# haliphinx/TCE-RVOS

Measured on AMD Instinct MI355X. Metric: clips/s (T=5, 360×640, Swin-T) at 1/2/4/8 MI355X; mask IoU vs ref, higher is better.
Workload: dtype f32 (3xf16-split MFMA, f32 accumulate); 1 GPU; swin_t_p4w7 T=5 360x640 + 32-token text, B=1 clip per forward, flags --with_box_refine --binary --f_token 8 --qtrans (BASELINE config 2); clips_in_flight_per_gpu=1, clips_per_forward=1, same_clip_in_group=False, ranks_per_gpu=1, parallelism=clip-sharded x1

## Files before the change

tce-rvos_amd/csrc/fewrow.hip:

```cpp
#include "common.h"
#include "../../include/tce_rvos.h"

namespace {

constexpr int FR_COLS = 8;
constexpr int FR_KC = 256;
constexpr int FR_PITCH = FR_KC + 4;

struct FrSegDev {
  const float* W;
  const float* bias;
  float* out;
  int N, ldw, ldo, use_a2, act, slab0;
};

struct FrArgs {
  const float* x;
  const float* a2;
  const float* res;
  long long ldx, lda2, ldres;
  int a2_rows, R, K, nseg;
  FrSegDev seg[3];
  const float *g_in, *be_in;
  float* xn_out;
  long long ldxn;
  float eps_in;
};

template <int RPT>
__global__ void __launch_bounds__(256) fewrow_linear_kernel(const FrArgs p) {
  __shared__ __attribute__((aligned(16))) float sX[32 * RPT * FR_PITCH];
  __shared__ __attribute__((aligned(16))) float sW[FR_COLS * FR_PITCH];
  const int tid = threadIdx.x;
  int s = 0;
  if (p.nseg > 1 && (int)blockIdx.x >= p.seg[1].slab0) s = 1;
  if (p.nseg > 2 && (int)blockIdx.x >= p.seg[2].slab0) s = 2;
  const FrSegDev sg = s == 0 ? p.seg[0] : (s == 1 ? p.seg[1] : p.seg[2]);
  const int n0 = ((int)blockIdx.x - sg.slab0) * FR_COLS;
  const int r0 = blockIdx.y * (32 * RPT);
  const int nr = min(32 * RPT, p.R - r0);
  const int c = tid & 7, g = tid >> 3;
  float acc[RPT];
#pragma unroll
  for (int i = 0; i < RPT; ++i) acc[i] = 0.f;
  for (int k0 = 0; k0 < p.K; k0 += FR_KC) {
    const int kc = min(FR_KC, p.K - k0);
    const int q4 = kc >> 2;
    if (k0) __syncthreads();
    if ((tid & 63) < q4) {
      const int q = tid & 63;
      for (int r = tid >> 6; r < 32 * RPT; r += 4) {
        f32x4 v = {0.f, 0.f, 0.f, 0.f};
        if (r < nr) {
          v = *reinterpret_cast<const f32x4*>(p.x + (long long)(r0 + r) * p.ldx + k0 + 4 * q);
          if (p.g_in) {
            const float mean = wave_sum((v[0] + v[1]) + (v[2] + v[3])) / (float)p.K;
            const f32x4 d = {v[0] - mean, v[1] - mean, v[2] - mean, v[3] - mean};
            const float rstd = rsqrtf(wave_sum(fmaf(d[0], d[0], fmaf(d[1], d[1], fmaf(d[2], d[2], d[3] * d[3])))) / (float)p.K + p.eps_in);
            const f32x4 g = *reinterpret_cast<const f32x4*>(p.g_in + 4 * q), b = *reinterpret_cast<const f32x4*>(p.be_in + 4 * q);
            v = f32x4{d[0] * rstd * g[0] + b[0], d[1] * rstd * g[1] + b[1], d[2] * rstd * g[2] + b[2], d[3] * rstd * g[3] + b[3]};
            if (p.xn_out && blockIdx.x == 0) *reinterpret_cast<f32x4*>(p.xn_out + (long long)(r0 + r) * p.ldxn + 4 * q) = v;
          }
          if (sg.use_a2) {
            const int ra = p.a2_rows > 0 ? (r0 + r) % p.a2_rows : r0 + r;
            v += *reinterpret_cast<const f32x4*>(p.a2 + (long long)ra * p.lda2 + k0 + 4 * q);
          }
        }
        *reinterpret_cast<f32x4*>(&sX[r * FR_PITCH + 4 * q]) = v;
      }
      for (int r = tid >> 6; r < FR_COLS; r += 4) {
        f32x4 v = {0.f, 0.f, 0.f, 0.f};
        if (n0 + r < sg.N) v = *reinterpret_cast<const f32x4*>(sg.W + (long long)(n0 + r) * sg.ldw + k0 + 4 * q);
        *reinterpret_cast<f32x4*>(&sW[r * FR_PITCH + 4 * q]) = v;
      }
    }
    __syncthreads();
    const float* wrow = &sW[c * FR_PITCH];
    const float* xrow = &sX[g * FR_PITCH];
    if (q4 == 64) {
#pragma unroll 8
      for (int q = 0; q < 64; ++q) {
        const f32x4 wv = *reinterpret_cast<const f32x4*>(wrow + 4 * q);
#pragma unroll
        for (int i = 0; i < RPT; ++i) {
          const f32x4 xv = *reinterpret_cast<const f32x4*>(xrow + i * 32 * FR_PITCH + 4 * q);
          acc[i] = fmaf(xv[0], wv[0], acc[i]);
          acc[i] = fmaf(xv[1], wv[1], acc[i]);
          acc[i] = fmaf(xv[2], wv[2], acc[i]);
          acc[i] = fmaf(xv[3], wv[3], acc[i]);
        }
      }
    } else {
      for (int q = 0; q < q4; ++q) {
        const f32x4 wv = *reinterpret_cast<const f32x4*>(wrow + 4 * q);
#pragma unroll
        for (int i = 0; i < RPT; ++i) {
          const f32x4 xv = *reinterpret_cast<const f32x4*>(xrow + i * 32 * FR_PITCH + 4 * q);
          acc[i] = fmaf(xv[0], wv[0], acc[i]);
          acc[i] = fmaf(xv[1], wv[1], acc[i]);
          acc[i] = fmaf(xv[2], wv[2], acc[i]);
          acc[i] = fmaf(xv[3], wv[3], acc[i]);
        }
      }
    }
  }
  const int n = n0 + c;
  if (n < sg.N) {
    const float bv = sg.bias ? sg.bias[n] : 0.f;
#pragma unroll
    for (int i = 0; i < RPT; ++i) {
      const int r = g + 32 * i;
      if (r < nr) {
        float v = acc[i] + bv;
        if (sg.act == 1) v = fmaxf(v, 0.f);
        if (sg.act == 2) v = 1.0f / (1.0f + __expf(-v));
        if (sg.act == 3) v = tce_gelu(v);
        if (s == 0 && p.res) v += p.res[(long long)(r0 + r) * p.ldres + n];
        sg.out[(long long)(r0 + r) * sg.ldo + n] = v;
      }
    }
  }
}

}

extern "C" int tce_fewrow_linear_f32(const tceFewRowArgs* a, tceStream stream) {
  TCE_CHECK_ARG(a && a->x && a->nseg >= 1 && a->nseg <= 3, "tce_fewrow_linear_f32: bad arguments");
  TCE_CHECK_ARG(a->R > 0 && a->K > 0 && a->K % 4 == 0 && a->ldx % 4 == 0 && a->ldx >= a->K && tce_aligned16(a->x),
                "tce_fewrow_linear_f32: K and ldx must be multiples of 4, ldx >= K, x 16-byte aligned");
  auto span = [&](const float* p, long long ld, long long cols, long long rows, const float*& b, const float*& e) {
    b = p;
    e = p + (rows - 1) * ld + cols;
  };
  auto disjoint = [](const float* b0, const float* e0, const float* b1, const float* e1) { return e0 <= b1 || e1 <= b0; };
  FrArgs p;
  p.g_in = a->g_in; p.be_in = a->be_in; p.xn_out = a->g_in ? a->xn_out : nullptr; p.ldxn = a->ldxn; p.eps_in = a->eps_in;
  if (a->g_in) {
    TCE_CHECK_ARG(a->be_in && a->K == FR_KC && tce_aligned16(a->g_in) && tce_aligned16(a->be_in),
                  "tce_fewrow_linear_f32: the LayerNorm prologue needs K = %d and 16-byte aligned gamma / beta", FR_KC);
    TCE_CHECK_ARG(!a->xn_out || (a->ldxn >= a->K && a->ldxn % 4 == 0 && tce_aligned16(a->xn_out)), "tce_fewrow_linear_f32: xn_out pitch / alignment");
  }
  p.x = a->x; p.a2 = a->a2; p.res = a->res;
  p.ldx = a->ldx; p.lda2 = a->lda2; p.ldres = a->ldres;
  p.a2_rows = a->a2_rows; p.R = a->R; p.K = a->K; p.nseg = a->nseg;
  int slabs = 0;
  for (int s = 0; s < 3; ++s) {
    FrSegDev& d = p.seg[s];
    d = FrSegDev{nullptr, nullptr, nullptr, 0, 0, 0, 0, 0, 1 << 30};
    if (s >= a->nseg) continue;
    const tceFewRowSeg& g = a->seg[s];
    TCE_CHECK_ARG(g.W && g.out && g.N > 0 && g.ldw % 4 == 0 && g.ldw >= a->K && g.ldo >= g.N && tce_aligned16(g.W),
                  "tce_fewrow_linear_f32: segment %d: bad weight / output geometry", s);
    TCE_CHECK_ARG(!g.use_a2 || (a->a2 && a->lda2 % 4 == 0 && tce_aligned16(a->a2)), "tce_fewrow_linear_f32: addend missing / misaligned");
    TCE_CHECK_ARG(g.act >= 0 && g.act <= 3, "tce_fewrow_linear_f32: act must be 0 (none), 1 (ReLU), 2 (sigmoid) or 3 (GELU)");
    {
      const float *xb, *xe, *ob, *oe;
      span(a->x, a->ldx, a->K, a->R, xb, xe);
      span(g.out, g.ldo, g.N, a->R, ob, oe);
      TCE_CHECK_ARG(disjoint(xb, xe, ob, oe), "tce_fewrow_linear_f32: segment %d: out overlaps x", s);
      if (a->a2) {
        const float *ab, *ae;
        span(a->a2, a->lda2, a->K, a->a2_rows > 0 ? a->a2_rows : a->R, ab, ae);
        TCE_CHECK_ARG(disjoint(ab, ae, ob, oe), "tce_fewrow_linear_f32: segment %d: out overlaps a2", s);
      }
      for (int t = 0; t < s; ++t) {
        const float *pb, *pe;
        span(a->seg[t].out, a->seg[t].ldo, a->seg[t].N, a->R, pb, pe);
        TCE_CHECK_ARG(disjoint(pb, pe, ob, oe), "tce_fewrow_linear_f32: outputs of segments %d and %d overlap", t, s);
      }
      if (a->g_in && a->xn_out) {
        const float *nb, *ne;
        span(a->xn_out, a->ldxn, a->K, a->R, nb, ne);
        TCE_CHECK_ARG(disjoint(nb, ne, xb, xe) && disjoint(nb, ne, ob, oe), "tce_fewrow_linear_f32: xn_out overlaps x or segment %d's out", s);
        if (a->a2) {
          const float *ab, *ae;
          span(a->a2, a->lda2, a->K, a->a2_rows > 0 ? a->a2_rows : a->R, ab, ae);
          TCE_CHECK_ARG(disjoint(nb, ne, ab, ae), "tce_fewrow_linear_f32: xn_out overlaps a2");
        }
      }
      if (a->res) {
        const float *rb, *re;
        span(a->res, a->ldres, a->seg[0].N, a->R, rb, re);
        const bool in_place = s == 0 && a->res == g.out && a->ldres == g.ldo;
        TCE_CHECK_ARG(in_place || disjoint(rb, re, ob, oe),
                      "tce_fewrow_linear_f32: segment %d: res overlaps out (only segment 0 may alias it, exactly)", s);
      }
    }
    d.W = g.W; d.bias = g.bias; d.out = g.out; d.N = g.N; d.ldw = g.ldw; d.ldo = g.ldo; d.use_a2 = g.use_a2; d.act = g.act;
    d.slab0 = slabs;
    slabs += tce_cdiv(g.N, FR_COLS);
  }
  TCE_CHECK_ARG(!a->res || a->ldres >= a->seg[0].N, "tce_fewrow_linear_f32: residual pitch");
#ifdef FEWROW_RPT2
  if (a->R > 32 && a->R <= 64) {
    hipLaunchKernelGGL(fewrow_linear_kernel<2>, dim3(slabs, 1), dim3(256), 0, (hipStream_t)stream, p);
    TCE_CHECK_LAUNCH("tce_fewrow_linear_f32");
    return TCE_OK;
  }
#endif
  hipLaunchKernelGGL(fewrow_linear_kernel<1>, dim3(slabs, tce_cdiv(a->R, 32)), dim3(256), 0, (hipStream_t)stream, p);
  TCE_CHECK_LAUNCH("tce_fewrow_linear_f32");
  return TCE_OK;
}
```

tce-rvos_amd/csrc/ffn.hip:

```cpp
#include "common.h"
#include "gemm_epilogue.h"
#include "frag.h"
#include "tiles.h"
#include "../../include/tce_rvos.h"
#include "../../include/tce_rvos_debug.h"

namespace {

#ifndef FFN_ABL
#define FFN_ABL 0
#endif
static __device__ long long* g_ffn_stamps = nullptr;

__device__ __forceinline__ void partial_store(const f32x16& acc, float* __restrict__ base, const int t, const int lane) {
#pragma unroll
  for (int g = 0; g < 4; ++g) {
    const f32x4 o = {acc[4 * g], acc[4 * g + 1], acc[4 * g + 2], acc[4 * g + 3]};
    float* const ptr = base + ((t * 4 + g) * 64 + lane) * 4;
    asm volatile("global_store_dwordx4 %0, %1, off sc1" ::"v"(ptr), "v"(o) : "memory");
  }
}
struct PartTile {
  f32x4 v[4];
};
// ... 429 lines not shown
    o = __builtin_bit_cast(u32x4, plane ? f.lo : f.hi);
  }
  reinterpret_cast<u32x4*>(out)[u] = o;
}

inline bool ffn_shape_ok(int C, int Hd) { return (C == 96 || C == 128 || C == 192 || C == 256) && Hd > 0 && Hd % 32 == 0; }
inline int ffn_waves(int C) { return C <= 128 ? 8 : 4; }
inline int ffn_pieces(int C) {
  const int w = ffn_waves(C);
  return (1 + 2 * (C / 16) + 4 * (C / 32) + w - 1) / w * w;
}
inline long long ffn_units(int C, int Hd) { return (long long)(Hd / 32 + 2) * ffn_pieces(C) * 64; }

struct FfnSplitPlan {
  int p = 0, k[2] = {0, 0}, nblk = 0;
  long long ws_floats = 0;
};
inline FfnSplitPlan ffn_split_plan(int M, int C, int Hd, int batch) {
  FfnSplitPlan best;
  const int B = tce_cdiv(M, 32 * ffn_waves(C)), NC = Hd / 32, CUS = tce_cu_count();
  if (C != 256 || NC < 24 || batch < 1) return best;
  const int OVP = 3, OVF = 4;
  auto rounds = [&](long long wgs) { return (double)((wgs + CUS - 1) / CUS); };
  double best_cost = 0.75 * rounds((long long)B * batch) * (NC + 1 + OVP + OVF);
  for (int p = 1; p <= 2; ++p) {
    const int wd = p == 1 ? 0 : (p * NC - 2 * (1 + OVP)) / (p + 1), ws_ = p == 1 ? (NC + 1) / 2 : wd + 1 + OVP;
    int k[2] = {ws_, 0};
    bool ok = ws_ >= 1 && ws_ <= NC - 1;
    for (int i = 1; i < p && ok; ++i) {
      k[i] = wd - (NC - k[i - 1]);
      ok = k[i] >= 1 && k[i] <= NC - 1;
    }
    if (!ok) continue;
    const int busiest = ws_ > NC - k[p - 1] ? ws_ : NC - k[p - 1];
    const double cost = rounds((long long)tce_cdiv(B, p) * (p + 1) * batch) * (busiest + 1 + OVP + OVF);
    if (cost < best_cost) {
      best_cost = cost;
      best.p = p;
      for (int i = 0; i < 2; ++i) best.k[i] = k[i];
    }
  }
  if (best.p) {
    best.nblk = B;
    best.ws_floats = (long long)batch * B * 2 * (32 * ffn_waves(C)) * C;
  }
  return best;
}

static int g_ffn_half = 0;

struct FfnGridPlan {
  int grid_x, persist;
};
inline FfnGridPlan ffn_grid_plan(int cap, int batch, int blocks) {
  if (cap <= 0 || batch < 1 || (long long)blocks * batch <= cap) return {blocks, 0};
  const int gx = cap / batch > 1 ? cap / batch : 1;
  if (gx >= blocks) return {blocks, 0};
  return {gx, 1};
}
static thread_local int t_ffn_wg_cap = 0;

template <int C, int WAVES>
void ffn_launch(const FfnArgs& a, int act, hipStream_t s, int batch = 1) {
  if constexpr (C == 256) {
    if (a.sp_p > 0 && act == 1) {
      const dim3 grid(tce_cdiv(a.nblk, a.sp_p) * (a.sp_p + 1), batch), block(64 * WAVES);
      if (a.single) hipLaunchKernelGGL((ffn_fused_kernel<C, WAVES, 1, true, 0, true>), grid, block, 0, s, a);
      else hipLaunchKernelGGL((ffn_fused_kernel<C, WAVES, 1, false, 0, true>), grid, block, 0, s, a);
      return;
    }
  }
  if constexpr (C <= 128 && WAVES == 8) {
    const long long b8 = (long long)tce_cdiv(a.M, 256) * batch, b4 = (long long)tce_cdiv(a.M, 128) * batch, cus = tce_cu_count();
    const double c8 = (double)((b8 + cus - 1) / cus);
    const long long rem = b4 % (2 * cus);
    const double c4 = (double)(b4 / (2 * cus)) + (rem == 0 ? 0.0 : rem <= cus ? 0.5 : 1.0);
    if (act == 2 && g_ffn_half >= 0 && (g_ffn_half > 0 || c4 <= c8)) {
      const dim3 grid(tce_cdiv(a.M, 128), batch), block(256);
      if (a.single) hipLaunchKernelGGL((ffn_fused_kernel<C, 4, 2, true>), grid, block, 0, s, a);
      else hipLaunchKernelGGL((ffn_fused_kernel<C, 4, 2, false>), grid, block, 0, s, a);
      return;
    }
  }
  if constexpr (C == 256) {
    const FfnGridPlan gp = ffn_grid_plan(t_ffn_wg_cap, batch, tce_cdiv(a.M, 32 * WAVES));
    if (gp.persist && act == 1) {
      const dim3 grid(gp.grid_x, batch), block(64 * WAVES);
      if (a.single) hipLaunchKernelGGL((ffn_fused_kernel<C, WAVES, 1, true, 0, false, true>), grid, block, 0, s, a);
      else hipLaunchKernelGGL((ffn_fused_kernel<C, WAVES, 1, false, 0, false, true>), grid, block, 0, s, a);
      return;
    }
  }
  const dim3 grid(tce_cdiv(a.M, 32 * WAVES), batch), block(64 * WAVES);
  if (a.single) {
    if (act == 1) hipLaunchKernelGGL((ffn_fused_kernel<C, WAVES, 1, true>), grid, block, 0, s, a);
    else if (act == 2) hipLaunchKernelGGL((ffn_fused_kernel<C, WAVES, 2, true>), grid, block, 0, s, a);
  } else {
    if (act == 1) hipLaunchKernelGGL((ffn_fused_kernel<C, WAVES, 1, false>), grid, block, 0, s, a);
    else if (act == 2) hipLaunchKernelGGL((ffn_fused_kernel<C, WAVES, 2, false>), grid, block, 0, s, a);
  }
}

__global__ void __launch_bounds__(256) xattn_prepare_kernel(const float* __restrict__ k, const float* __restrict__ v,
                                                            const float* __restrict__ wqT, const float* __restrict__ wo,
                                                            float* __restrict__ W1, float* __restrict__ b1,
                                                            float* __restrict__ W2, const int L, const int G,
                                                            const int* __restrict__ lens) {
  constexpr int C = 256, HD = 32;
  const int Hd = 8 * G;
  const int Lb = lens ? min(lens[blockIdx.y], L) : L;
  k += (long long)blockIdx.y * L * C;
  v += (long long)blockIdx.y * L * C;
  W1 += (long long)blockIdx.y * Hd * C;
  b1 += (long long)blockIdx.y * Hd;
  W2 += (long long)blockIdx.y * C * Hd;
  const int idx = blockIdx.x * 256 + threadIdx.x;
  if (idx < Hd * C) {
    const int r = idx / C, i = idx - r * C, h = r / G, j = r - h * G;
    float a = 0.f;
    if (j < Lb) {
      const f32x4* kp = reinterpret_cast<const f32x4*>(k + j * C + h * HD);
      const f32x4* wp = reinterpret_cast<const f32x4*>(wqT + (long long)i * C + h * HD);
#pragma unroll
      for (int c4 = 0; c4 < 8; ++c4) {
        const f32x4 kv = kp[c4], wv = wp[c4];
        a = fmaf(kv[0], wv[0], a); a = fmaf(kv[1], wv[1], a); a = fmaf(kv[2], wv[2], a); a = fmaf(kv[3], wv[3], a);
      }
    }
    W1[idx] = a;
  } else if (idx < 2 * Hd * C) {
    const int e = idx - Hd * C, n = e / Hd, r = e - n * Hd, h = r / G, j = r - h * G;
    float a = 0.f;
    if (j < Lb) {
      const f32x4* vp = reinterpret_cast<const f32x4*>(v + j * C + h * HD);
      const f32x4* wp = reinterpret_cast<const f32x4*>(wo + (long long)n * C + h * HD);
#pragma unroll
      for (int c4 = 0; c4 < 8; ++c4) {
        const f32x4 vv = vp[c4], wv = wp[c4];
        a = fmaf(vv[0], wv[0], a); a = fmaf(vv[1], wv[1], a); a = fmaf(vv[2], wv[2], a); a = fmaf(vv[3], wv[3], a);
      }
    }
    W2[e] = a;
  } else if (idx < 2 * Hd * C + Hd) {
    const int r = idx - 2 * Hd * C, h = r / G, j = r - h * G;
    float a = -1.0e30f;
    if (j < Lb) {
      a = 0.f;
      for (int c = 0; c < HD; ++c) a = fmaf(k[j * C + h * HD + c], wqT[(long long)C * C + h * HD + c], a);
    }
    b1[r] = a;
  }
}

__global__ void __launch_bounds__(256) xattn_pack_fused_kernel(const float* __restrict__ k, const float* __restrict__ v,
                                                               const float* __restrict__ wqT, const float* __restrict__ wo,
                                                               unsigned char* __restrict__ out, const int L, const int G,
                                                               const int P, const int SL, const long long threads,
                                                               const long long units, const int single,
                                                               const int* __restrict__ lens) {
  constexpr int C = 256, HD = 32, KS = C / 16, NT = C / 32;
  const long long tix = (long long)blockIdx.x * 256 + threadIdx.x;
  if (tix >= threads) return;
  const int Hd = 8 * G, NC = Hd / 32;
  const int Lb = lens ? min(lens[blockIdx.y], L) : L;
  k += (long long)blockIdx.y * L * C;
  v += (long long)blockIdx.y * L * C;
  out += (long long)blockIdx.y * units * 16;
  const int lane = (int)(tix & 63);
  const long long sg = tix >> 6;
  const int sl = (int)(sg % SL), it = (int)(sg / SL);
  const int r = lane & 31, hf = lane >> 5;
  u32x4* const stage_out = reinterpret_cast<u32x4*>(out) + (long long)it * P * 64;
  auto dot32 = [](const float* a, const float* b) {
    const f32x4* ap = reinterpret_cast<const f32x4*>(a);
    const f32x4* bp = reinterpret_cast<const f32x4*>(b);
    float acc = 0.f;
#pragma unroll
    for (int c4 = 0; c4 < 8; ++c4) {
      const f32x4 x = ap[c4], y = bp[c4];
      acc = fmaf(x[0], y[0], acc); acc = fmaf(x[1], y[1], acc); acc = fmaf(x[2], y[2], acc); acc = fmaf(x[3], y[3], acc);
    }
    return acc;
  };
  if (sl == 0) {
    u32x4 o = {0u, 0u, 0u, 0u};
    if (lane < 8 && it < NC) {
      f32x4 val;
#pragma unroll
      for (int c = 0; c < 4; ++c) {
        const int idx = 4 * lane + c, h2 = idx >> 4, i = idx & 15;
        const int row = 32 * it + (i & 3) + 8 * (i >> 2) + 4 * h2, h = row / G, j = row - h * G;
        float a = -1.0e30f;
        if (j < Lb) {
          a = 0.f;
          for (int c2 = 0; c2 < HD; ++c2) a = fmaf(k[j * C + h * HD + c2], wqT[(long long)C * C + h * HD + c2], a);
        }
        val[c] = a;
      }
      o = __builtin_bit_cast(u32x4, val);
    }
    stage_out[lane] = o;
    return;
  }
  const int p_hi = 2 * sl - 1, p_lo = 2 * sl;
  if (p_hi >= P) return;
  u32x4 oh = {0u, 0u, 0u, 0u}, ol = oh;
  if (p_hi < 1 + 2 * KS + 4 * NT) {
    float val[8];
    if (p_hi <= 2 * KS) {
      const int s = (p_hi - 1) >> 1;
      const int row = 32 * it + r, h = row / G, j = row - h * G;
#pragma unroll
      for (int e = 0; e < 8; ++e)
        val[e] = (it < NC && j < Lb) ? dot32(k + j * C + h * HD, wqT + (long long)(16 * s + 8 * hf + e) * C + h * HD) : 0.f;
    } else {
      const int idx = (p_hi - 1 - 2 * KS) >> 1, t = idx >> 1, s2 = idx & 1, chunk = it - 1;
#pragma unroll
      for (int e = 0; e < 8; ++e) {
        const int col = 32 * chunk + 16 * s2 + 8 * (e >> 2) + 4 * hf + (e & 3);
        const int h = col / G, j = col - h * G;
        val[e] = (chunk >= 0 && chunk < NC && j < Lb) ? dot32(wo + (long long)(32 * t + r) * C + h * HD, v + j * C + h * HD) : 0.f;
      }
    }
    const HL f = split8(val, single);
    oh = __builtin_bit_cast(u32x4, f.hi);
    ol = __builtin_bit_cast(u32x4, f.lo);
  }
  stage_out[p_hi * 64 + lane] = oh;
  if (p_lo < P) stage_out[p_lo * 64 + lane] = ol;
}

}

extern "C" int tce_debug_ffn_set_stamp_buffer(long long* dev_buf) {
  if (tce_rowlin_set_stamps(dev_buf) != 0) return -1;
  return hipMemcpyToSymbol(HIP_SYMBOL(g_ffn_stamps), &dev_buf, sizeof(dev_buf)) == hipSuccess ? 0 : -1;
}

extern "C" int64_t tce_ffn_packed_bytes(int32_t C, int32_t Hd) { return ffn_shape_ok(C, Hd) ? ffn_units(C, Hd) * 16 : -1; }

extern "C" int tce_ffn_pack_f32(const float* W1, const float* b1, const float* W2, void* packed, int32_t C, int32_t Hd,
                                tceStream stream) {
  TCE_CHECK_ARG(ffn_shape_ok(C, Hd), "tce_ffn_pack_f32: unsupported shape C=%d hidden=%d (C in 96/128/192/256, hidden %% 32 == 0)",
                C, Hd);
  TCE_CHECK_ARG(W1 && W2 && packed && tce_aligned16(packed), "tce_ffn_pack_f32: null / misaligned pointer");
  const long long units = ffn_units(C, Hd);
  hipLaunchKernelGGL(ffn_pack_kernel, dim3(tce_cdiv(units, 256)), dim3(256), 0, (hipStream_t)stream, W1, b1, W2,
                     (unsigned char*)packed, C, Hd, ffn_pieces(C), units, tce_gemm_single_pass());
  TCE_CHECK_LAUNCH("tce_ffn_pack_f32");
  return TCE_OK;
}

extern "C" int tce_ffn_pack_batched_f32(const float* W1, const float* b1, const float* W2, void* packed, int32_t C, int32_t Hd,
                                        int32_t batch, tceStream stream) {
  TCE_CHECK_ARG(ffn_shape_ok(C, Hd) && batch > 0, "tce_ffn_pack_batched_f32: unsupported shape C=%d hidden=%d batch=%d", C, Hd, batch);
  TCE_CHECK_ARG(W1 && W2 && packed && tce_aligned16(packed), "tce_ffn_pack_batched_f32: null / misaligned pointer");
  const long long units = ffn_units(C, Hd);
  hipLaunchKernelGGL(ffn_pack_kernel, dim3(tce_cdiv(units, 256), batch), dim3(256), 0, (hipStream_t)stream, W1, b1, W2,
                     (unsigned char*)packed, C, Hd, ffn_pieces(C), units, tce_gemm_single_pass());
  TCE_CHECK_LAUNCH("tce_ffn_pack_batched_f32");
  return TCE_OK;
}

extern "C" int tce_ffn_pack_chain_f32(const float* W1, const float* b1, const float* W2, void* packed, int32_t C, int32_t Hd,
                                      tceStream stream) {
  TCE_CHECK_ARG(C == 256 && ffn_shape_ok(C, Hd), "tce_ffn_pack_chain_f32: C must be 256, hidden %% 32 == 0 (C=%d hidden=%d)", C, Hd);
  TCE_CHECK_ARG(W1 && W2 && packed && tce_aligned16(packed), "tce_ffn_pack_chain_f32: null / misaligned pointer");
  const long long units = ffn_units(C, Hd);
  hipLaunchKernelGGL(ffn_pack_kernel, dim3(tce_cdiv(units, 256)), dim3(256), 0, (hipStream_t)stream, W1, b1, W2,
                     (unsigned char*)packed, C, Hd, ffn_pieces(C), units, tce_gemm_single_pass(), 1);
  TCE_CHECK_LAUNCH("tce_ffn_pack_chain_f32");
  return TCE_OK;
}

extern "C" int tce_ffn_fused_f32(const float* x, int64_t ldx, const void* packed, const float* b2, const float* g_in,
                                 const float* be_in, float eps_in, const float* g_out, const float* be_out,
                                 float eps_out, float* out, int64_t ldo, int32_t M, int32_t C, int32_t Hd, int32_t act,
                                 tceStream stream) {
  TCE_CHECK_ARG(ffn_shape_ok(C, Hd), "tce_ffn_fused_f32: unsupported shape C=%d hidden=%d", C, Hd);
  TCE_CHECK_ARG(M > 0 && x && packed && b2 && out, "tce_ffn_fused_f32: null pointer or M <= 0");
  TCE_CHECK_ARG(act == 1 || act == 2, "tce_ffn_fused_f32: act must be 1 (ReLU) or 2 (GELU)");
  TCE_CHECK_ARG(ldx >= C && ldo >= C && ldx % 4 == 0 && ldo % 4 == 0, "tce_ffn_fused_f32: bad row pitch");
  TCE_CHECK_ARG(tce_aligned16(x) && tce_aligned16(out) && tce_aligned16(packed) && tce_aligned16(b2),
                "tce_ffn_fused_f32: x/out/packed/b2 must be 16-byte aligned");
  TCE_CHECK_ARG((!g_in || (be_in && tce_aligned16(g_in) && tce_aligned16(be_in))) &&
                    (!g_out || (be_out && tce_aligned16(g_out) && tce_aligned16(be_out))),
                "tce_ffn_fused_f32: LayerNorm gamma/beta must come in pairs, 16-byte aligned");
  FfnArgs a = {};
  a.x = x; a.wpk = (const unsigned char*)packed; a.b2 = b2; a.res_mode = 1;
  a.g_in = g_in; a.be_in = be_in; a.g_out = g_out; a.be_out = be_out;
  a.out = out; a.ldx = ldx; a.ldo = ldo; a.M = M; a.NI = Hd / 32 + 1; a.eps_in = eps_in; a.eps_out = eps_out; a.range_flag = tce_range_flag(); a.single = tce_gemm_single_pass();
  a.wdiv = 1;
  hipStream_t s = (hipStream_t)stream;
  if (C == 256) ffn_launch<256, 4>(a, act, s);
  else if (C == 192) ffn_launch<192, 4>(a, act, s);
  else if (C == 128) ffn_launch<128, 8>(a, act, s);
  else ffn_launch<96, 8>(a, act, s);
  TCE_CHECK_LAUNCH("tce_ffn_fused_f32");
  return TCE_OK;
}

extern "C" int tce_ffn_set_wg_cap(int32_t cap) {
  TCE_CHECK_ARG(cap >= 0, "tce_ffn_set_wg_cap: cap must be >= 0 (0 = none)");
  t_ffn_wg_cap = cap;
  return TCE_OK;
}

extern "C" int32_t tce_ffn_capped_grid(int32_t cap, int32_t batch, int32_t blocks, int32_t* persistent) {
  const FfnGridPlan gp = ffn_grid_plan(cap, batch, blocks);
  if (persistent) *persistent = gp.persist;
  return gp.grid_x;
}

extern "C" int tce_debug_ffn_set_half(int32_t mode) {
  TCE_CHECK_ARG(mode >= -1 && mode <= 1, "tce_debug_ffn_set_half: -1 (never), 0 (automatic) or 1 (always)");
  g_ffn_half = mode;
  return TCE_OK;
}

extern "C" int64_t tce_ffn_split_ws_floats(int32_t M, int32_t C, int32_t Hd, int32_t act) {
  if (M <= 0 || !ffn_shape_ok(C, Hd) || act != 1) return 0;
  return ffn_split_plan(M, C, Hd, 1).ws_floats;
}

extern "C" int32_t tce_ffn_split_counters(int32_t M, int32_t C, int32_t Hd, int32_t act) {
  if (M <= 0 || !ffn_shape_ok(C, Hd) || act != 1) return 0;
  return ffn_split_plan(M, C, Hd, 1).nblk;
}

extern "C" int tce_ffn_fused_split_f32(const float* x, int64_t ldx, const void* packed, const float* b2, const float* g_in,
                                       const float* be_in, float eps_in, const float* g_out, const float* be_out, float eps_out,
                                       float* out, int64_t ldo, int32_t M, int32_t C, int32_t Hd, int32_t act, float* ws,
                                       int64_t ws_floats, int32_t* counters, int32_t n_counters, tceStream stream) {
  TCE_CHECK_ARG(ffn_shape_ok(C, Hd), "tce_ffn_fused_split_f32: unsupported shape C=%d hidden=%d", C, Hd);
  TCE_CHECK_ARG(M > 0 && x && packed && b2 && out, "tce_ffn_fused_split_f32: null pointer or M <= 0");
  TCE_CHECK_ARG(act == 1, "tce_ffn_fused_split_f32: act must be 1 (ReLU)");
  TCE_CHECK_ARG(ldx >= C && ldo >= C && ldx % 4 == 0 && ldo % 4 == 0, "tce_ffn_fused_split_f32: bad row pitch");
  TCE_CHECK_ARG(tce_aligned16(x) && tce_aligned16(out) && tce_aligned16(packed) && tce_aligned16(b2),
                "tce_ffn_fused_split_f32: x/out/packed/b2 must be 16-byte aligned");
  TCE_CHECK_ARG((!g_in || (be_in && tce_aligned16(g_in) && tce_aligned16(be_in))) &&
                    (!g_out || (be_out && tce_aligned16(g_out) && tce_aligned16(be_out))),
                "tce_ffn_fused_split_f32: LayerNorm gamma/beta must come in pairs, 16-byte aligned");
  const FfnSplitPlan plan = ffn_split_plan(M, C, Hd, 1);
  TCE_CHECK_ARG(plan.p > 0, "tce_ffn_fused_split_f32: no split is planned for M=%d C=%d hidden=%d (tce_ffn_split_ws_floats is 0): "
                "call tce_ffn_fused_f32", M, C, Hd);
  TCE_CHECK_ARG(ws && tce_aligned16(ws) && ws_floats >= plan.ws_floats && counters && n_counters >= plan.nblk,
                "tce_ffn_fused_split_f32: workspace of %lld floats and %d zeroed counters needed", plan.ws_floats, plan.nblk);
  TCE_CHECK_ARG(!(ws <= out + (long long)(M - 1) * ldo + C - 1 && out <= ws + plan.ws_floats - 1) &&
                    !(ws <= x + (long long)(M - 1) * ldx + C - 1 && x <= ws + plan.ws_floats - 1),
                "tce_ffn_fused_split_f32: the workspace overlaps x / out");
  FfnArgs a = {};
  a.x = x; a.wpk = (const unsigned char*)packed; a.b2 = b2; a.res_mode = 1;
  a.g_in = g_in; a.be_in = be_in; a.g_out = g_out; a.be_out = be_out;
  a.out = out; a.ldx = ldx; a.ldo = ldo; a.M = M; a.NI = Hd / 32 + 1; a.eps_in = eps_in; a.eps_out = eps_out; a.range_flag = tce_range_flag(); a.single = tce_gemm_single_pass();
  a.wdiv = 1;
  a.ws = ws; a.cnt = counters; a.sp_p = plan.p; a.sp_k0 = plan.k[0]; a.sp_k1 = plan.k[1]; a.nblk = plan.nblk;
  ffn_launch<256, 4>(a, act, (hipStream_t)stream);
  TCE_CHECK_LAUNCH("tce_ffn_fused_split_f32");
  return TCE_OK;
}

extern "C" int tce_xattn_prepare_f32(const float* k, const float* v, const float* wqT_ext, const float* wo, float* W1, float* b1,
                                     float* W2, int32_t L, int32_t group, int32_t batch, tceStream stream) {
  TCE_CHECK_ARG(k && v && wqT_ext && wo && W1 && b1 && W2, "tce_xattn_prepare_f32: null pointer");
  TCE_CHECK_ARG((group == 32 || group == 8) && L >= 1 && L <= group && batch >= 1,
                "tce_xattn_prepare_f32: group must be 32 or 8 and 1 <= L <= group (L=%d group=%d)", L, group);
  TCE_CHECK_ARG(tce_aligned16(k) && tce_aligned16(v) && tce_aligned16(wqT_ext) && tce_aligned16(wo),
                "tce_xattn_prepare_f32: pointers must be 16-byte aligned");
  const int Hd = 8 * group;
  hipLaunchKernelGGL(xattn_prepare_kernel, dim3(tce_cdiv(2 * Hd * 256 + Hd, 256), batch), dim3(256), 0, (hipStream_t)stream,
                     k, v, wqT_ext, wo, W1, b1, W2, L, group, (const int*)nullptr);
  TCE_CHECK_LAUNCH("tce_xattn_prepare_f32");
  return TCE_OK;
}

extern "C" int tce_xattn_pack_f32(const float* k, const float* v, const float* wqT_ext, const float* wo, void* packed, int32_t L,
                                  int32_t group, int32_t batch, tceStream stream) {
  TCE_CHECK_ARG(k && v && wqT_ext && wo && packed, "tce_xattn_pack_f32: null pointer");
  TCE_CHECK_ARG((group == 32 || group == 8) && L > 0 && L <= group && batch > 0, "tce_xattn_pack_f32: group must be 32 or 8, 0 < L <= group");
  TCE_CHECK_ARG(tce_aligned16(k) && tce_aligned16(v) && tce_aligned16(wqT_ext) && tce_aligned16(wo) && tce_aligned16(packed),
                "tce_xattn_pack_f32: pointers must be 16-byte aligned");
  const int Hd = 8 * group;
  const long long units = ffn_units(256, Hd);
  const int P = ffn_pieces(256), SL = 1 + P / 2;
  const long long threads = (long long)(Hd / 32 + 2) * SL * 64;
  hipLaunchKernelGGL(xattn_pack_fused_kernel, dim3(tce_cdiv(threads, 256), batch), dim3(256), 0, (hipStream_t)stream, k, v, wqT_ext,
                     wo, (unsigned char*)packed, L, group, P, SL, threads, units, tce_gemm_single_pass(), (const int*)nullptr);
  TCE_CHECK_LAUNCH("tce_xattn_pack_f32");
  return TCE_OK;
}

extern "C" int tce_xattn_prepare_lens_f32(const float* k, const float* v, const float* wqT_ext, const float* wo, float* W1, float* b1,
                                          float* W2, int32_t L, int32_t group, int32_t batch, const int32_t* lens, tceStream stream) {
  TCE_CHECK_ARG(k && v && wqT_ext && wo && W1 && b1 && W2 && lens, "tce_xattn_prepare_lens_f32: null pointer");
  TCE_CHECK_ARG((group == 32 || group == 8) && L >= 1 && L <= group && batch >= 1,
                "tce_xattn_prepare_lens_f32: group must be 32 or 8 and 1 <= L <= group (L=%d group=%d)", L, group);
  TCE_CHECK_ARG(tce_aligned16(k) && tce_aligned16(v) && tce_aligned16(wqT_ext) && tce_aligned16(wo),
                "tce_xattn_prepare_lens_f32: pointers must be 16-byte aligned");
  const int Hd = 8 * group;
  hipLaunchKernelGGL(xattn_prepare_kernel, dim3(tce_cdiv(2 * Hd * 256 + Hd, 256), batch), dim3(256), 0, (hipStream_t)stream,
                     k, v, wqT_ext, wo, W1, b1, W2, L, group, (const int*)lens);
  TCE_CHECK_LAUNCH("tce_xattn_prepare_lens_f32");
  return TCE_OK;
}

extern "C" int tce_xattn_pack_lens_f32(const float* k, const float* v, const float* wqT_ext, const float* wo, void* packed, int32_t L,
                                       int32_t group, int32_t batch, const int32_t* lens, tceStream stream) {
  TCE_CHECK_ARG(k && v && wqT_ext && wo && packed && lens, "tce_xattn_pack_lens_f32: null pointer");
  TCE_CHECK_ARG((group == 32 || group == 8) && L > 0 && L <= group && batch > 0,
                "tce_xattn_pack_lens_f32: group must be 32 or 8, 0 < L <= group");
  TCE_CHECK_ARG(tce_aligned16(k) && tce_aligned16(v) && tce_aligned16(wqT_ext) && tce_aligned16(wo) && tce_aligned16(packed),
                "tce_xattn_pack_lens_f32: pointers must be 16-byte aligned");
  const int Hd = 8 * group;
  const long long units = ffn_units(256, Hd);
  const int P = ffn_pieces(256), SL = 1 + P / 2;
  const long long threads = (long long)(Hd / 32 + 2) * SL * 64;
  hipLaunchKernelGGL(xattn_pack_fused_kernel, dim3(tce_cdiv(threads, 256), batch), dim3(256), 0, (hipStream_t)stream, k, v, wqT_ext,
                     wo, (unsigned char*)packed, L, group, P, SL, threads, units, tce_gemm_single_pass(), (const int*)lens);
  TCE_CHECK_LAUNCH("tce_xattn_pack_lens_f32");
  return TCE_OK;
}

static int xattn_launch(const tceXattnArgs* args, const tceXattnFfnArgs* ffn, tceStream stream);

extern "C" int tce_xattn_fused_f32(const tceXattnArgs* args, tceStream stream) { return xattn_launch(args, nullptr, stream); }

extern "C" int tce_xattn_ffn_fused_f32(const tceXattnArgs* args, const tceXattnFfnArgs* ffn, tceStream stream) {
  TCE_CHECK_ARG(args && ffn, "tce_xattn_ffn_fused_f32: null args");
  TCE_CHECK_ARG(ffn->packed && ffn->b2 && ffn->mid && ffn->hidden > 0 && ffn->hidden % 32 == 0 && ffn_shape_ok(256, ffn->hidden),
                "tce_xattn_ffn_fused_f32: bad FFN stage (packed / b2 / mid / hidden)");
  TCE_CHECK_ARG(ffn->act == 1, "tce_xattn_ffn_fused_f32: the FFN stage's activation must be 1 (ReLU)");
  TCE_CHECK_ARG(ffn->ldmid >= 256 && ffn->ldmid % 4 == 0 && ffn->sMid % 4 == 0 && tce_aligned16(ffn->mid) && tce_aligned16(ffn->packed) &&
                    tce_aligned16(ffn->b2) && (!ffn->g_out || (ffn->be_out && tce_aligned16(ffn->g_out) && tce_aligned16(ffn->be_out))),
                "tce_xattn_ffn_fused_f32: FFN stage pitch / alignment");
  TCE_CHECK_ARG(args->res_mode == 1, "tce_xattn_ffn_fused_f32: the attention stage's residual must be additive");
  TCE_CHECK_ARG(ffn->mid != args->x && ffn->mid != args->out && ffn->mid != args->res,
                "tce_xattn_ffn_fused_f32: mid must be a buffer of its own (it is written and re-read inside the launch)");
  return xattn_launch(args, ffn, stream);
}

static int xattn_launch(const tceXattnArgs* args, const tceXattnFfnArgs* ffn, tceStream stream) {
  TCE_CHECK_ARG(args != nullptr, "tce_xattn_fused_f32: null args");
  const tceXattnArgs& q = *args;
  TCE_CHECK_ARG(q.M > 0 && q.x && q.packed && q.bo && q.out, "tce_xattn_fused_f32: null pointer or M <= 0");
  TCE_CHECK_ARG(q.res_mode == 1 || q.res_mode == 2, "tce_xattn_fused_f32: res_mode must be 1 (add) or 2 (multiply)");
  TCE_CHECK_ARG(q.group == 32 || q.group == 8, "tce_xattn_fused_f32: group (key slots per head) must be 32 or 8");
  TCE_CHECK_ARG(q.ldx >= 256 && q.ldo >= 256 && q.ldx % 4 == 0 && q.ldo % 4 == 0 && (!q.res || (q.ldres >= 256 && q.ldres % 4 == 0)) &&
                    (!q.a2 || (q.lda2 >= 256 && q.lda2 % 4 == 0)) && q.sX % 4 == 0 && q.sRes % 4 == 0 && q.sOut % 4 == 0,
                "tce_xattn_fused_f32: bad row pitch / batch stride");
  TCE_CHECK_ARG(tce_aligned16(q.x) && tce_aligned16(q.out) && tce_aligned16(q.packed) && tce_aligned16(q.bo) &&
                    (!q.a2 || tce_aligned16(q.a2)) && (!q.res || tce_aligned16(q.res)),
                "tce_xattn_fused_f32: pointers must be 16-byte aligned");
  TCE_CHECK_ARG(!q.g_out || (q.be_out && tce_aligned16(q.g_out) && tce_aligned16(q.be_out)),
                "tce_xattn_fused_f32: LayerNorm gamma/beta must come in pairs, 16-byte aligned");
  FfnArgs a = {};
  a.x = q.x; a.wpk = (const unsigned char*)q.packed; a.b2 = q.bo; a.g_out = q.g_out; a.be_out = q.be_out; a.out = q.out;
  a.ldx = q.ldx; a.ldo = q.ldo; a.a2 = q.a2; a.lda2 = q.lda2; a.a2_rows = q.a2_rows; a.res = q.res; a.ldres = q.ldres;
  a.res_mode = q.res_mode; a.sX = q.sX; a.sRes = q.sRes; a.sOut = q.sOut; a.sW = q.sW;
  a.M = q.M; a.NI = (8 * q.group) / 32 + 1; a.eps_out = q.eps_out; a.range_flag = tce_range_flag(); a.single = tce_gemm_single_pass();
  a.wdiv = q.w_div > 0 ? q.w_div : 1;
  const int batch = q.batch > 0 ? q.batch : 1;
  const dim3 grid(tce_cdiv(a.M, 128), batch), block(256);
  if (ffn) {
    a.wpk2 = (const unsigned char*)ffn->packed; a.b22 = ffn->b2; a.g_out2 = ffn->g_out; a.be_out2 = ffn->be_out; a.eps_out2 = ffn->eps_out;
    a.mid = ffn->mid; a.ldmid = ffn->ldmid; a.sMid = ffn->sMid; a.NI2 = ffn->hidden / 32 + 1;
    if (a.single) {
      if (q.group == 32) hipLaunchKernelGGL((ffn_fused_kernel<256, 4, 3, true, 1>), grid, block, 0, (hipStream_t)stream, a);
      else hipLaunchKernelGGL((ffn_fused_kernel<256, 4, 4, true, 1>), grid, block, 0, (hipStream_t)stream, a);
    } else {
      if (q.group == 32) hipLaunchKernelGGL((ffn_fused_kernel<256, 4, 3, false, 1>), grid, block, 0, (hipStream_t)stream, a);
      else hipLaunchKernelGGL((ffn_fused_kernel<256, 4, 4, false, 1>), grid, block, 0, (hipStream_t)stream, a);
    }
    TCE_CHECK_LAUNCH("tce_xattn_ffn_fused_f32");
    return TCE_OK;
  }
  const FfnGridPlan gp = ffn_grid_plan(t_ffn_wg_cap, batch, tce_cdiv(a.M, 128));
  if (gp.persist) {
    const dim3 pgrid(gp.grid_x, batch);
    if (a.single) {
      if (q.group == 32) hipLaunchKernelGGL((ffn_fused_kernel<256, 4, 3, true, 0, false, true>), pgrid, block, 0, (hipStream_t)stream, a);
      else hipLaunchKernelGGL((ffn_fused_kernel<256, 4, 4, true, 0, false, true>), pgrid, block, 0, (hipStream_t)stream, a);
    } else {
      if (q.group == 32) hipLaunchKernelGGL((ffn_fused_kernel<256, 4, 3, false, 0, false, true>), pgrid, block, 0, (hipStream_t)stream, a);
      else hipLaunchKernelGGL((ffn_fused_kernel<256, 4, 4, false, 0, false, true>), pgrid, block, 0, (hipStream_t)stream, a);
    }
    TCE_CHECK_LAUNCH("tce_xattn_fused_f32");
    return TCE_OK;
  }
  if (a.single) {
    if (q.group == 32) hipLaunchKernelGGL((ffn_fused_kernel<256, 4, 3, true>), grid, block, 0, (hipStream_t)stream, a);
    else hipLaunchKernelGGL((ffn_fused_kernel<256, 4, 4, true>), grid, block, 0, (hipStream_t)stream, a);
  } else {
    if (q.group == 32) hipLaunchKernelGGL((ffn_fused_kernel<256, 4, 3, false>), grid, block, 0, (hipStream_t)stream, a);
    else hipLaunchKernelGGL((ffn_fused_kernel<256, 4, 4, false>), grid, block, 0, (hipStream_t)stream, a);
  }
  TCE_CHECK_LAUNCH("tce_xattn_fused_f32");
  return TCE_OK;
}
```

Baseline: 169.0 clips/s.

## Stage xattn pack weights in LDS and prefetch fewrow operands before barrier

```diff
diff --git a/tce-rvos_amd/csrc/fewrow.hip b/tce-rvos_amd/csrc/fewrow.hip
--- a/tce-rvos_amd/csrc/fewrow.hip
+++ b/tce-rvos_amd/csrc/fewrow.hip
@@ -4,6 +4,8 @@
 namespace {
 
 constexpr int FR_COLS = 8;
+constexpr int FR_NT = 32 * FR_COLS;
+constexpr int FR_WAVES = FR_NT / 64;
 constexpr int FR_KC = 256;
 constexpr int FR_PITCH = FR_KC + 4;
 
@@ -28,8 +30,9 @@
 };
 
 template <int RPT>
-__global__ void __launch_bounds__(256) fewrow_linear_kernel(const FrArgs p) {
-  __shared__ __attribute__((aligned(16))) float sX[32 * RPT * FR_PITCH];
+__global__ void __launch_bounds__(FR_NT) fewrow_linear_kernel(const FrArgs p) {
+  constexpr int ROWS = 32 * RPT, XR = ROWS / FR_WAVES, WR = FR_COLS / FR_WAVES;
+  __shared__ __attribute__((aligned(16))) float sX[ROWS * FR_PITCH];
   __shared__ __attribute__((aligned(16))) float sW[FR_COLS * FR_PITCH];
   const int tid = threadIdx.x;
   int s = 0;
@@ -37,76 +40,96 @@
   if (p.nseg > 2 && (int)blockIdx.x >= p.seg[2].slab0) s = 2;
   const FrSegDev sg = s == 0 ? p.seg[0] : (s == 1 ? p.seg[1] : p.seg[2]);
   const int n0 = ((int)blockIdx.x - sg.slab0) * FR_COLS;
-  const int r0 = blockIdx.y * (32 * RPT);
-  const int nr = min(32 * RPT, p.R - r0);
-  const int c = tid & 7, g = tid >> 3;
+  const int r0 = blockIdx.y * ROWS;
+  const int nr = min(ROWS, p.R - r0);
+  const int c = tid % FR_COLS, g = tid / FR_COLS;
+  const int n = n0 + c;
+  float bv = 0.f, rv[RPT];
+#pragma unroll
+  for (int i = 0; i < RPT; ++i) {
+    const int r = g + 32 * i;
+    rv[i] = (n < sg.N && r < nr && s == 0 && p.res) ? p.res[(long long)(r0 + r) * p.ldres + n] : 0.f;
+  }
+  if (n < sg.N && sg.bias) bv = sg.bias[n];
   float acc[RPT];
 #pragma unroll
   for (int i = 0; i < RPT; ++i) acc[i] = 0.f;
+  const int q = tid & 63, w = tid >> 6;
   for (int k0 = 0; k0 < p.K; k0 += FR_KC) {
     const int kc = min(FR_KC, p.K - k0);
     const int q4 = kc >> 2;
+    const f32x4 zero = {0.f, 0.f, 0.f, 0.f};
+    f32x4 wv[WR], xv[XR], av[XR];
+    if (q < q4) {
+#pragma unroll
+      for (int i = 0; i < WR; ++i) {
+        const int r = w + FR_WAVES * i;
+        wv[i] = n0 + r < sg.N ? *reinterpret_cast<const f32x4*>(sg.W + (long long)(n0 + r) * sg.ldw + k0 + 4 * q) : zero;
+      }
+#pragma unroll
+      for (int i = 0; i < XR; ++i) {
+        const int r = w + FR_WAVES * i;
+        xv[i] = r < nr ? *reinterpret_cast<const f32x4*>(p.x + (long long)(r0 + r) * p.ldx + k0 + 4 * q) : zero;
+        av[i] = zero;
+        if (sg.use_a2 && r < nr) {
+          const int ra = p.a2_rows > 0 ? (r0 + r) % p.a2_rows : r0 + r;
+          av[i] = *reinterpret_cast<const f32x4*>(p.a2 + (long long)ra * p.lda2 + k0 + 4 * q);
+        }
+      }
+    }
     if (k0) __syncthreads();
-    if ((tid & 63) < q4) {
-      const int q = tid & 63;
-      for (int r = tid >> 6; r < 32 * RPT; r += 4) {
-        f32x4 v = {0.f, 0.f, 0.f, 0.f};
+    if (q < q4) {
+#pragma unroll
+      for (int i = 0; i < XR; ++i) {
+        const int r = w + FR_WAVES * i;
+        f32x4 v = xv[i];
         if (r < nr) {
-          v = *reinterpret_cast<const f32x4*>(p.x + (long long)(r0 + r) * p.ldx + k0 + 4 * q);
           if (p.g_in) {
             const float mean = wave_sum((v[0] + v[1]) + (v[2] + v[3])) / (float)p.K;
             const f32x4 d = {v[0] - mean, v[1] - mean, v[2] - mean, v[3] - mean};
             const float rstd = rsqrtf(wave_sum(fmaf(d[0], d[0], fmaf(d[1], d[1], fmaf(d[2], d[2], d[3] * d[3])))) / (float)p.K + p.eps_in);
-            const f32x4 g = *reinterpret_cast<const f32x4*>(p.g_in + 4 * q), b = *reinterpret_cast<const f32x4*>(p.be_in + 4 * q);
-            v = f32x4{d[0] * rstd * g[0] + b[0], d[1] * rstd * g[1] + b[1], d[2] * rstd * g[2] + b[2], d[3] * rstd * g[3] + b[3]};
+            const f32x4 ga = *reinterpret_cast<const f32x4*>(p.g_in + 4 * q), b = *reinterpret_cast<const f32x4*>(p.be_in + 4 * q);
+            v = f32x4{d[0] * rstd * ga[0] + b[0], d[1] * rstd * ga[1] + b[1], d[2] * rstd * ga[2] + b[2], d[3] * rstd * ga[3] + b[3]};
             if (p.xn_out && blockIdx.x == 0) *reinterpret_cast<f32x4*>(p.xn_out + (long long)(r0 + r) * p.ldxn + 4 * q) = v;
           }
-          if (sg.use_a2) {
-            const int ra = p.a2_rows > 0 ? (r0 + r) % p.a2_rows : r0 + r;
-            v += *reinterpret_cast<const f32x4*>(p.a2 + (long long)ra * p.lda2 + k0 + 4 * q);
-          }
+          if (sg.use_a2) v += av[i];
         }
         *reinterpret_cast<f32x4*>(&sX[r * FR_PITCH + 4 * q]) = v;
       }
-      for (int r = tid >> 6; r < FR_COLS; r += 4) {
-        f32x4 v = {0.f, 0.f, 0.f, 0.f};
-        if (n0 + r < sg.N) v = *reinterpret_cast<const f32x4*>(sg.W + (long long)(n0 + r) * sg.ldw + k0 + 4 * q);
-        *reinterpret_cast<f32x4*>(&sW[r * FR_PITCH + 4 * q]) = v;
-      }
+#pragma unroll
+      for (int i = 0; i < WR; ++i) *reinterpret_cast<f32x4*>(&sW[(w + FR_WAVES * i) * FR_PITCH + 4 * q]) = wv[i];
     }
     __syncthreads();
     const float* wrow = &sW[c * FR_PITCH];
     const float* xrow = &sX[g * FR_PITCH];
     if (q4 == 64) {
 #pragma unroll 8
-      for (int q = 0; q < 64; ++q) {
-        const f32x4 wv = *reinterpret_cast<const f32x4*>(wrow + 4 * q);
+      for (int qq = 0; qq < 64; ++qq) {
+        const f32x4 wq = *reinterpret_cast<const f32x4*>(wrow + 4 * qq);
 #pragma unroll
         for (int i = 0; i < RPT; ++i) {
-          const f32x4 xv = *reinterpret_cast<const f32x4*>(xrow + i * 32 * FR_PITCH + 4 * q);
-          acc[i] = fmaf(xv[0], wv[0], acc[i]);
-          acc[i] = fmaf(xv[1], wv[1], acc[i]);
-          acc[i] = fmaf(xv[2], wv[2], acc[i]);
-          acc[i] = fmaf(xv[3], wv[3], acc[i]);
+          const f32x4 xq = *reinterpret_cast<const f32x4*>(xrow + i * 32 * FR_PITCH + 4 * qq);
+          acc[i] = fmaf(xq[0], wq[0], acc[i]);
+          acc[i] = fmaf(xq[1], wq[1], acc[i]);
+          acc[i] = fmaf(xq[2], wq[2], acc[i]);
+          acc[i] = fmaf(xq[3], wq[3], acc[i]);
         }
       }
     } else {
-      for (int q = 0; q < q4; ++q) {
-        const f32x4 wv = *reinterpret_cast<const f32x4*>(wrow + 4 * q);
+      for (int qq = 0; qq < q4; ++qq) {
+        const f32x4 wq = *reinterpret_cast<const f32x4*>(wrow + 4 * qq);
 #pragma unroll
         for (int i = 0; i < RPT; ++i) {
-          const f32x4 xv = *reinterpret_cast<const f32x4*>(xrow + i * 32 * FR_PITCH + 4 * q);
-          acc[i] = fmaf(xv[0], wv[0], acc[i]);
-          acc[i] = fmaf(xv[1], wv[1], acc[i]);
-          acc[i] = fmaf(xv[2], wv[2], acc[i]);
-          acc[i] = fmaf(xv[3], wv[3], acc[i]);
-        }
-      }
-    }
-  }
-  const int n = n0 + c;
+          const f32x4 xq = *reinterpret_cast<const f32x4*>(xrow + i * 32 * FR_PITCH + 4 * qq);
+          acc[i] = fmaf(xq[0], wq[0], acc[i]);
+          acc[i] = fmaf(xq[1], wq[1], acc[i]);
+          acc[i] = fmaf(xq[2], wq[2], acc[i]);
+          acc[i] = fmaf(xq[3], wq[3], acc[i]);
+        }
+      }
+    }
+  }
   if (n < sg.N) {
-    const float bv = sg.bias ? sg.bias[n] : 0.f;
 #pragma unroll
     for (int i = 0; i < RPT; ++i) {
       const int r = g + 32 * i;
@@ -115,7 +138,7 @@
         if (sg.act == 1) v = fmaxf(v, 0.f);
         if (sg.act == 2) v = 1.0f / (1.0f + __expf(-v));
         if (sg.act == 3) v = tce_gelu(v);
-        if (s == 0 && p.res) v += p.res[(long long)(r0 + r) * p.ldres + n];
+        if (s == 0 && p.res) v += rv[i];
         sg.out[(long long)(r0 + r) * sg.ldo + n] = v;
       }
     }
@@ -193,12 +216,12 @@
   TCE_CHECK_ARG(!a->res || a->ldres >= a->seg[0].N, "tce_fewrow_linear_f32: residual pitch");
 #ifdef FEWROW_RPT2
   if (a->R > 32 && a->R <= 64) {
-    hipLaunchKernelGGL(fewrow_linear_kernel<2>, dim3(slabs, 1), dim3(256), 0, (hipStream_t)stream, p);
+    hipLaunchKernelGGL(fewrow_linear_kernel<2>, dim3(slabs, 1), dim3(FR_NT), 0, (hipStream_t)stream, p);
     TCE_CHECK_LAUNCH("tce_fewrow_linear_f32");
     return TCE_OK;
   }
 #endif
-  hipLaunchKernelGGL(fewrow_linear_kernel<1>, dim3(slabs, tce_cdiv(a->R, 32)), dim3(256), 0, (hipStream_t)stream, p);
+  hipLaunchKernelGGL(fewrow_linear_kernel<1>, dim3(slabs, tce_cdiv(a->R, 32)), dim3(FR_NT), 0, (hipStream_t)stream, p);
   TCE_CHECK_LAUNCH("tce_fewrow_linear_f32");
   return TCE_OK;
 }
diff --git a/tce-rvos_amd/csrc/ffn.hip b/tce-rvos_amd/csrc/ffn.hip
--- a/tce-rvos_amd/csrc/ffn.hip
+++ b/tce-rvos_amd/csrc/ffn.hip
@@ -605,25 +605,29 @@
   }
 }
 
+constexpr int XP_KV_PITCH = 36;
+constexpr int XP_W_PITCH_MAX = 4 * XP_KV_PITCH + 4;
+static_assert(XP_KV_PITCH % 4 == 0 && XP_W_PITCH_MAX % 4 == 0, "lines are addressed in float4");
+
 __global__ void __launch_bounds__(256) xattn_pack_fused_kernel(const float* __restrict__ k, const float* __restrict__ v,
                                                                const float* __restrict__ wqT, const float* __restrict__ wo,
                                                                unsigned char* __restrict__ out, const int L, const int G,
-                                                               const int P, const int SL, const long long threads,
-                                                               const long long units, const int single,
+                                                               const int P, const long long units, const int single,
                                                                const int* __restrict__ lens) {
   constexpr int C = 256, HD = 32, KS = C / 16, NT = C / 32;
-  const long long tix = (long long)blockIdx.x * 256 + threadIdx.x;
-  if (tix >= threads) return;
+  __shared__ f32x4 sm[(64 * XP_W_PITCH_MAX + 32 * XP_KV_PITCH) / 4];
+  constexpr int KV0 = 64 * XP_W_PITCH_MAX / 4, LP = XP_KV_PITCH / 4;
+  const int tid = threadIdx.x, lane = tid & 63, w = tid >> 6;
   const int Hd = 8 * G, NC = Hd / 32;
   const int Lb = lens ? min(lens[blockIdx.y], L) : L;
   k += (long long)blockIdx.y * L * C;
   v += (long long)blockIdx.y * L * C;
   out += (long long)blockIdx.y * units * 16;
-  const int lane = (int)(tix & 63);
-  const long long sg = tix >> 6;
-  const int sl = (int)(sg % SL), it = (int)(sg / SL);
+  const int it = (int)blockIdx.x / 9, q = (int)blockIdx.x % 9;
   const int r = lane & 31, hf = lane >> 5;
   u32x4* const stage_out = reinterpret_cast<u32x4*>(out) + (long long)it * P * 64;
+  const u32x4 zero = {0u, 0u, 0u, 0u};
+  auto fmac = [](float& acc, const float a, const float b) { asm("v_fmac_f32 %0, %1, %2" : "+v"(acc) : "v"(a), "v"(b)); };
   auto dot32 = [](const float* a, const float* b) {
     const f32x4* ap = reinterpret_cast<const f32x4*>(a);
     const f32x4* bp = reinterpret_cast<const f32x4*>(b);
@@ -635,52 +639,104 @@
     }
     return acc;
   };
-  if (sl == 0) {
-    u32x4 o = {0u, 0u, 0u, 0u};
-    if (lane < 8 && it < NC) {
-      f32x4 val;
-#pragma unroll
-      for (int c = 0; c < 4; ++c) {
-        const int idx = 4 * lane + c, h2 = idx >> 4, i = idx & 15;
-        const int row = 32 * it + (i & 3) + 8 * (i >> 2) + 4 * h2, h = row / G, j = row - h * G;
-        float a = -1.0e30f;
-        if (j < Lb) {
-          a = 0.f;
-          for (int c2 = 0; c2 < HD; ++c2) a = fmaf(k[j * C + h * HD + c2], wqT[(long long)C * C + h * HD + c2], a);
+  if (q == 8) {
+    if (w == 0) {
+      u32x4 o = zero;
+      if (lane < 8 && it < NC) {
+        f32x4 val;
+#pragma unroll
+        for (int c = 0; c < 4; ++c) {
+          const int idx = 4 * lane + c, h2 = idx >> 4, i = idx & 15;
+          const int row = 32 * it + (i & 3) + 8 * (i >> 2) + 4 * h2, h = row / G, j = row - h * G;
+          val[c] = j < Lb ? dot32(k + j * C + h * HD, wqT + (long long)C * C + h * HD) : -1.0e30f;
         }
-        val[c] = a;
-      }
-      o = __builtin_bit_cast(u32x4, val);
-    }
-    stage_out[lane] = o;
+        o = __builtin_bit_cast(u32x4, val);
+      }
+      stage_out[lane] = o;
+    } else {
+      const int piece = 2 * KS + 4 * NT + w;
+      if (piece < P) stage_out[piece * 64 + lane] = zero;
+    }
     return;
   }
-  const int p_hi = 2 * sl - 1, p_lo = 2 * sl;
-  if (p_hi >= P) return;
-  u32x4 oh = {0u, 0u, 0u, 0u}, ol = oh;
-  if (p_hi < 1 + 2 * KS + 4 * NT) {
-    float val[8];
-    if (p_hi <= 2 * KS) {
-      const int s = (p_hi - 1) >> 1;
-      const int row = 32 * it + r, h = row / G, j = row - h * G;
-#pragma unroll
-      for (int e = 0; e < 8; ++e)
-        val[e] = (it < NC && j < Lb) ? dot32(k + j * C + h * HD, wqT + (long long)(16 * s + 8 * hf + e) * C + h * HD) : 0.f;
-    } else {
-      const int idx = (p_hi - 1 - 2 * KS) >> 1, t = idx >> 1, s2 = idx & 1, chunk = it - 1;
-#pragma unroll
-      for (int e = 0; e < 8; ++e) {
-        const int col = 32 * chunk + 16 * s2 + 8 * (e >> 2) + 4 * hf + (e & 3);
-        const int h = col / G, j = col - h * G;
-        val[e] = (chunk >= 0 && chunk < NC && j < Lb) ? dot32(wo + (long long)(32 * t + r) * C + h * HD, v + j * C + h * HD) : 0.f;
-      }
-    }
-    const HL f = split8(val, single);
-    oh = __builtin_bit_cast(u32x4, f.hi);
-    ol = __builtin_bit_cast(u32x4, f.lo);
-  }
-  stage_out[p_hi * 64 + lane] = oh;
-  if (p_lo < P) stage_out[p_lo * 64 + lane] = ol;
+  const int sl = 1 + 4 * q + w, p_hi = 2 * sl - 1, p_lo = 2 * sl;
+  const bool w1 = q < 4;
+  const int chunk = w1 ? it : it - 1;
+  if (chunk < 0 || chunk >= NC) {
+    stage_out[p_hi * 64 + lane] = zero;
+    stage_out[p_lo * 64 + lane] = zero;
+    return;
+  }
+  const int nh = 32 / G, h0 = chunk * nh;
+  const int wpitch = nh > 1 ? nh * LP + 1 : LP, w4 = 8 * nh;
+  {
+    const float* const wsrc = (w1 ? wqT : wo) + (long long)(64 * (q & 3)) * C + h0 * HD;
+    const float* const kv = w1 ? k : v;
+    f32x4 wv[8], kvv = {0.f, 0.f, 0.f, 0.f};
+#pragma unroll
+    for (int i = 0; i < 8; ++i)
+      if (i < 2 * nh) {
+        const int idx = tid + 256 * i, row = idx / w4, c4 = idx - row * w4;
+        wv[i] = *reinterpret_cast<const f32x4*>(wsrc + (long long)row * C + 4 * c4);
+      }
+    const int kr = tid >> 3, kh = h0 + kr / G, kj = kr % G;
+    if (kj < Lb) kvv = *reinterpret_cast<const f32x4*>(kv + kj * C + kh * HD + 4 * (tid & 7));
+#pragma unroll
+    for (int i = 0; i < 8; ++i)
+      if (i < 2 * nh) {
+        const int idx = tid + 256 * i, row = idx / w4, c4 = idx - row * w4;
+        sm[row * wpitch + (c4 >> 3) * LP + (c4 & 7)] = wv[i];
+      }
+    sm[KV0 + kr * LP + (tid & 7)] = kvv;
+  }
+  __syncthreads();
+  int xo[2], yo[8];
+  bool keep[8];
+  if (w1) {
+    const int hl = r / G, j = r - hl * G;
+    xo[0] = xo[1] = KV0 + r * LP;
+#pragma unroll
+    for (int e = 0; e < 8; ++e) {
+      yo[e] = (16 * w + 8 * hf + e) * wpitch + hl * LP;
+      keep[e] = j < Lb;
+    }
+  } else {
+    const int cl0 = 16 * (w & 1) + 4 * hf, xrow = (32 * (w >> 1) + r) * wpitch;
+    xo[0] = xrow + (cl0 / G) * LP;
+    xo[1] = xrow + ((cl0 + 8) / G) * LP;
+#pragma unroll
+    for (int e = 0; e < 8; ++e) {
+      const int cl = cl0 + 8 * (e >> 2) + (e & 3);
+      yo[e] = KV0 + cl * LP;
+      keep[e] = cl % G < Lb;
+    }
+  }
+  float val[8];
+#pragma unroll
+  for (int e = 0; e < 8; ++e) val[e] = 0.f;
+  f32x4 xb[2][2], yb[2][8];
+  auto fetch = [&](const int b, const int c4) {
+    xb[b][0] = sm[xo[0] + c4];
+    xb[b][1] = sm[xo[1] + c4];
+#pragma unroll
+    for (int e = 0; e < 8; ++e) yb[b][e] = sm[yo[e] + c4];
+  };
+  fetch(0, 0);
+#pragma unroll
+  for (int c4 = 0; c4 < 8; ++c4) {
+    if (c4 + 1 < 8) fetch((c4 + 1) & 1, c4 + 1);
+    __builtin_amdgcn_sched_barrier(0);
+#pragma unroll
+    for (int i = 0; i < 4; ++i)
+#pragma unroll
+      for (int e = 0; e < 8; ++e) fmac(val[e], xb[c4 & 1][e >> 2][i], yb[c4 & 1][e][i]);
+    __builtin_amdgcn_sched_barrier(0);
+  }
+#pragma unroll
+  for (int e = 0; e < 8; ++e) val[e] = keep[e] ? val[e] : 0.f;
+  const HL f = split8(val, single);
+  stage_out[p_hi * 64 + lane] = __builtin_bit_cast(u32x4, f.hi);
+  stage_out[p_lo * 64 + lane] = __builtin_bit_cast(u32x4, f.lo);
 }
 
 }
@@ -835,10 +891,9 @@
                 "tce_xattn_pack_f32: pointers must be 16-byte aligned");
   const int Hd = 8 * group;
   const long long units = ffn_units(256, Hd);
-  const int P = ffn_pieces(256), SL = 1 + P / 2;
-  const long long threads = (long long)(Hd / 32 + 2) * SL * 64;
-  hipLaunchKernelGGL(xattn_pack_fused_kernel, dim3(tce_cdiv(threads, 256), batch), dim3(256), 0, (hipStream_t)stream, k, v, wqT_ext,
-                     wo, (unsigned char*)packed, L, group, P, SL, threads, units, tce_gemm_single_pass(), (const int*)nullptr);
+  const int P = ffn_pieces(256);
+  hipLaunchKernelGGL(xattn_pack_fused_kernel, dim3(9 * (Hd / 32 + 2), batch), dim3(256), 0, (hipStream_t)stream, k, v, wqT_ext,
+                     wo, (unsigned char*)packed, L, group, P, units, tce_gemm_single_pass(), (const int*)nullptr);
   TCE_CHECK_LAUNCH("tce_xattn_pack_f32");
   return TCE_OK;
 }
@@ -866,10 +921,9 @@
                 "tce_xattn_pack_lens_f32: pointers must be 16-byte aligned");
   const int Hd = 8 * group;
   const long long units = ffn_units(256, Hd);
-  const int P = ffn_pieces(256), SL = 1 + P / 2;
-  const long long threads = (long long)(Hd / 32 + 2) * SL * 64;
-  hipLaunchKernelGGL(xattn_pack_fused_kernel, dim3(tce_cdiv(threads, 256), batch), dim3(256), 0, (hipStream_t)stream, k, v, wqT_ext,
-                     wo, (unsigned char*)packed, L, group, P, SL, threads, units, tce_gemm_single_pass(), (const int*)lens);
+  const int P = ffn_pieces(256);
+  hipLaunchKernelGGL(xattn_pack_fused_kernel, dim3(9 * (Hd / 32 + 2), batch), dim3(256), 0, (hipStream_t)stream, k, v, wqT_ext,
+                     wo, (unsigned char*)packed, L, group, P, units, tce_gemm_single_pass(), (const int*)lens);
   TCE_CHECK_LAUNCH("tce_xattn_pack_lens_f32");
   return TCE_OK;
 }
```

Result: no change. 170.2 clips/s, median of 6 (+0.7%).
